# endernewton/tf-faster-rcnn

Hardware: AMD Instinct MI355X
Metric: images/sec (600×1000) ResNet-101 Faster R-CNN at 1/2/4/8 MI355X (higher is better)
Workload: dtype f32 (operands, accumulators, results; GEMMs with Cin, Cout % 128 == 0 form each f32 product from two-piece fp16 operands with an exact power-of-two scale per 128-k block on the fp16 matrix pipe -- 3 MFMAs / product, dropped terms <= 3 * 2^-22, measured error vs float64 below the f32-MFMA kernel's; o

## Files before the change

### include/frcnn_hip.h

```cpp
#ifndef FRCNN_HIP_H_
#define FRCNN_HIP_H_
#include <stddef.h>
#include <stdint.h>

#ifdef __cplusplus
extern "C" {
#endif

#define FRCNN_OK 0
#define FRCNN_E_ARG (-1)
#define FRCNN_E_WS (-2)
#define FRCNN_E_UNSUPPORTED (-3)
#define FRCNN_E_HIP(e) (-(1000 + (int)(e)))

#define FRCNN_NMS_RULE_CPU 0
#define FRCNN_NMS_RULE_GPU 1

#define FRCNN_ACT_NONE 0
#define FRCNN_ACT_RELU 1
#define FRCNN_ACT_RELU6 2

#define FRCNN_ABI_VERSION 6
int frcnn_abi_version(void);
const char* frcnn_build_info(void);
// ... 178 lines not shown
                       const float* res_d, const void* res_planes_d, const float* res_inv_d, int G, int M, int N, int K, int act, int rows,
                       float* mean_out_d, void* ws, size_t ws_bytes, int cfg, void* stream);
int frcnn_winograd_filter_transform(const float* w_hwio, int Cin, int Cout, const float* scale, int m, float* u_out);
int frcnn_winograd_filter_transform_device(const float* w_packed_d, int Cout, int Cin, int m, int transpose_flip, float* u_d,
                                           void* stream);
int frcnn_winograd_input_transform(const float* x_d, int N, int H, int W, int C, int m, float* v_d, void* stream);
int frcnn_winograd_output_transform(const float* m_d, int N, int H, int W, int C, int m, const float* bias_d, int act, float* y_d,
                                    void* stream);
int frcnn_winograd2_conv_x3(const float* x_d, int N, int H, int W, const void* u_planes_d, const float* bias_d, int act, float* y_d,
                            void* stream);
int frcnn_winograd7_filter_transform(const float* w_hwio, int Cin, int Cout, const float* scale, float* u_out);
int frcnn_winograd7_filter_transform_device(const float* w_packed_d, int Cout, int Cin, int transpose_flip, float* u_d, void* stream);
int frcnn_winograd7_input_transform(const float* x_d, int R, int C, float* v_d, void* stream);
int frcnn_winograd7_output_transform(const float* m_d, int R, int C, const float* bias_d, int act, float* y_d, void* stream);
int frcnn_winograd_input_transform_h2(const float* x_d, int N, int H, int W, int C, int m, void* v_planes_d, float* v_inv_d, void* stream);
int frcnn_winograd_output_transform_h2(const float* m_d, int N, int H, int W, int C, int m, const float* bias_d, int act, float* y_d,
                                       void* y_planes_d, float* y_inv_d, void* stream);
int frcnn_winograd7_input_transform_h2(const float* x_d, int R, int C, void* v_planes_d, float* v_inv_d, void* stream);
int frcnn_winograd7_output_transform_h2(const float* m_d, int R, int C, const float* bias_d, int act, float* y_d, void* y_planes_d,
                                        float* y_inv_d, void* stream);
int frcnn_pack_filter_hwio(const float* w_hwio, int KH, int KW, int Cin, int Cout, const float* scale, float* out);
int frcnn_maxpool_nhwc(const float* x_d, int N, int H, int W, int C, int k, int stride, int pad_top,
                       int pad_left, float* y_d, int OH, int OW, void* stream);
int frcnn_dwconv3x3_nhwc(const float* x_d, int N, int H, int W, int C, const float* w_d, const float* bias_d,
                         float* y_d, int OH, int OW, int stride, int pad_top, int pad_left, int act, void* stream);
int frcnn_dwconv3x3_nhwc_h2(const float* x_d, int N, int H, int W, int C, const float* w_d, const float* bias_d, float* y_d,
                            void* y_planes_d, float* y_inv_d, int OH, int OW, int stride, int pad_top, int pad_left, int act, void* stream);
int frcnn_spatial_mean(const float* x_d, int N, int HW, int C, float* y_d, void* stream);
int frcnn_softmax_rows(const float* x_d, int R, int C, int ld, float* y_d, void* stream);
int frcnn_rpn_softmax(const float* score_d, int HW, int A, int ld, float* prob_d, void* stream);
int frcnn_copy_cols(const float* src_d, int R, int ld_src, int col0, int cols, float* dst_d, int ld_dst, void* stream);

size_t frcnn_anchor_target_workspace_bytes(int H, int W, int A, int max_gt);
int frcnn_anchor_target_layer(const float* gt_boxes_d, int G, float im_h, float im_w, int H, int W, int A,
                              int feat_stride, const double* base_d, int rpn_batchsize, double fg_fraction,
                              double pos_overlap, double neg_overlap, long long seed, const double* opts, float* labels_d,
                              float* bbox_targets_d, float* inside_w_d, float* outside_w_d, void* ws,
                              size_t ws_bytes, void* stream);
int frcnn_anchor_target_layer_inject(const float* gt_boxes_d, int G, float im_h, float im_w, int H, int W, int A, int feat_stride,
                                     const double* base_d, int rpn_batchsize, double fg_fraction, double pos_overlap,
                                     double neg_overlap, const int* disable_d, int n_disable, const double* opts, float* labels_d,
                                     float* bbox_targets_d, float* inside_w_d, float* outside_w_d, void* ws, size_t ws_bytes,
                                     void* stream);
int frcnn_proposal_target_layer(const float* rpn_rois_d, const float* rpn_scores_d, int N, const float* gt_boxes_d,
                                int G, int num_classes, int batch_size, double fg_fraction, double fg_thresh,
                                double bg_thresh_hi, double bg_thresh_lo, const double* means4, const double* stds4,
// ... 98 lines not shown
```

### tf-faster-rcnn_amd/csrc/conv_igemm.hip

```cpp
#include "common.h"
#include "mfma_f32.h"
#include <mutex>
#include <type_traits>

__device__ float4 g_zero_page[4];

struct ConvParams {
  const float* x; const float* w; const float* bias; const float* res; float* y;
  const float* mask;
  int N, H, W, Cin, OH, OW, Cout, KH, KW, stride, pad_top, pad_left, act;
  int RH, RW, res_stride;
  int M, Ktot, nsteps;
  int mtiles, ntiles;
  int batch;
  long long gx, gw, gy;
  int reserved;
  int splits, kchunk;
  long long gz;
  int stagger, stagger_slots;
};

__device__ __forceinline__ size_t res_offset_strided(int m, int n, int Cout, int res_stride, int ohow, int OW, int RH, int RW) {
  const int img = m / ohow, rem = m % ohow, oh = rem / OW, ow = rem % OW;
  return ((size_t)(img * RH + oh * res_stride) * RW + ow * res_stride) * Cout + n;
// ... 508 lines not shown
    case IGEMM_64x64_ILV: return launch_conv<64, 64, 32, 32, 2, false, true>(p, st);
    case IGEMM_128_RF: return launch_conv<128, 128, 64, 64, 2, false, false, true>(p, st);
    case IGEMM_128_8W_RF: return launch_conv<128, 128, 32, 64, 2, false, false, true>(p, st);
    case STREAM_64x64: return launch_stream<64, 64, 32, 32, true, false, false>(p, st);
    case STREAM_64x64_RESPF: return launch_stream<64, 64, 32, 32, true, false, true>(p, st);
    case STREAM_128_RF: return launch_stream<128, 128, 64, 64, false, true, false>(p, st);
    case STREAM_128_8W_RF: return launch_stream<128, 128, 32, 64, false, true, false>(p, st);
    case STREAM_128_8W_RF_RESPF: return launch_stream<128, 128, 32, 64, false, true, true>(p, st);
    case STREAM_128x64: return launch_stream<128, 64, 32, 32, true, false, false>(p, st);
    case STREAM_128x64_RESPF: return launch_stream<128, 64, 32, 32, true, false, true>(p, st);
    case STREAM_64x128: return launch_stream<64, 128, 32, 32, true, false, false>(p, st);
    case STREAM_64x128_RESPF: return launch_stream<64, 128, 32, 32, true, false, true>(p, st);
    case STREAM_128x64_4W_RESPF: return launch_stream<128, 64, 64, 32, false, true, true>(p, st);
    case STREAM_64x128_4W_RESPF: return launch_stream<64, 128, 32, 64, false, true, true>(p, st);
    case STREAM_32x64: return launch_stream<32, 64, 32, 32, true, false, false>(p, st);
    case STREAM_32x128: return launch_stream<32, 128, 32, 32, true, false, false>(p, st);
    default: return FRCNN_E_ARG;
  }
}

static thread_local int g_force_cfg = -1, g_stagger = 0, g_stream = 1, g_split_target = 640;
static thread_local int g_plan_images = 0;
static constexpr int PLAN_IMAGES = 4;
extern thread_local int g_wino_rows_below;
extern "C" int frcnn_set_tuning(int key, int value) {
  if (key == 9) { g_wino_rows_below = value > 0 ? value : 256; return FRCNN_OK; }
  if (key == 0) { g_force_cfg = value; return FRCNN_OK; }
  if (key == 5) { g_stagger = value; return FRCNN_OK; }
  if (key == 6) { g_stream = value; return FRCNN_OK; }
  if (key == 7) { g_split_target = value > 0 ? value : 640; return FRCNN_OK; }
  if (key == 8) { g_plan_images = value > 0 ? value : 0; return FRCNN_OK; }
  return FRCNN_E_ARG;
}

static long long plan_rows(long long M) {
  return (g_plan_images > 0 && M % g_plan_images == 0) ? M / g_plan_images * PLAN_IMAGES : M;
}

static long long tiles_128(long long rows, int Cout, int groups) { return (rows + 127) / 128 * cdiv(Cout, 128) * groups; }

static int tile_cfg_64(int Cout) { return Cout > 32 ? IGEMM_64x64_ILV : IGEMM_64x32_NS4; }
static int tile_cfg(long long rows, int Cout, int nsteps, int groups) {
  if (Cout >= 96 && tiles_128(rows, Cout, groups) >= 384 && nsteps >= 8) return Cout >= 1024 ? IGEMM_128_8W_RF : IGEMM_128_RF;
  return tile_cfg_64(Cout);
}

static bool short_k_stream(long long rows, int Cout, int nsteps, int groups) {
  return g_stream && nsteps <= 8 && Cout % 128 == 0 && (rows + 63) / 64 * (Cout / 128) * groups >= 512;
}

static int plan_splits(int M, int Cout, int nsteps) {
  if (g_force_cfg >= 0) return 1;
  M = (int)min(plan_rows(M), (long long)0x7fffffff);
  if (tile_cfg(M, Cout, nsteps, 1) != tile_cfg_64(Cout)) return 1;
// ... 110 lines not shown
                                 int Cout, int KH, int KW, int stride, int pad_top, int pad_left, int act, int fold_w,
                                 void* stream) {
  return conv2d_impl(x_d, N, H, W, Cin, w_d, bias_d, residual_d, RH, RW, res_stride, y_d, OH, OW, Cout, KH, KW, stride, pad_top,
                     pad_left, act, fold_w, nullptr, 0, nullptr, stream);
}

extern "C" int frcnn_conv2d_nhwc_ws(const float* x_d, int N, int H, int W, int Cin, const float* w_d, const float* bias_d,
                                    const float* residual_d, int RH, int RW, int res_stride, float* y_d, int OH, int OW,
                                    int Cout, int KH, int KW, int stride, int pad_top, int pad_left, int act, int fold_w,
                                    void* ws, size_t ws_bytes, void* stream) {
  return conv2d_impl(x_d, N, H, W, Cin, w_d, bias_d, residual_d, RH, RW, res_stride, y_d, OH, OW, Cout, KH, KW, stride, pad_top,
                     pad_left, act, fold_w, ws, ws_bytes, nullptr, stream);
}

extern "C" int frcnn_conv2d_nhwc_masked_ws(const float* x_d, int N, int H, int W, int Cin, const float* w_d, const float* bias_d,
                                           const float* residual_d, int RH, int RW, int res_stride, float* y_d, int OH, int OW,
                                           int Cout, int KH, int KW, int stride, int pad_top, int pad_left, int act, const float* mask_d,
                                           void* ws, size_t ws_bytes, void* stream) {
  if (!mask_d) return FRCNN_E_ARG;
  return conv2d_impl(x_d, N, H, W, Cin, w_d, bias_d, residual_d, RH, RW, res_stride, y_d, OH, OW, Cout, KH, KW, stride, pad_top,
                     pad_left, act, 0, ws, ws_bytes, mask_d, stream);
}

extern "C" int frcnn_gemm_batched_nt(const float* x_d, const float* w_d, float* y_d, int G, int M, int N, int K, void* stream) {
  if (!x_d || !w_d || !y_d || G <= 0 || M <= 0 || N <= 0 || K <= 0) return FRCNN_E_ARG;
  if (K % 32 || G > 65535) return FRCNN_E_UNSUPPORTED;
  ConvParams p = conv_params();
  p.x = x_d; p.w = w_d; p.y = y_d;
  p.N = 1; p.H = 1; p.W = M; p.Cin = K; p.OH = 1; p.OW = M; p.Cout = N;
  p.M = M; p.Ktot = K; p.nsteps = p.kchunk = K / 32;
  p.gx = (long long)M * K; p.gw = (long long)N * K; p.gy = (long long)M * N;
  p.batch = G;
  hipStream_t st = (hipStream_t)stream;
  if (g_force_cfg >= 0) return launch_cfg(g_force_cfg, p, st);
  const long long Mp = plan_rows(M);
  if (short_k_stream(Mp, N, p.nsteps, G)) {
    const int rc = launch_cfg(STREAM_64x128, p, st);
    if (rc != FRCNN_E_UNSUPPORTED) return rc;
  }
  const bool waste = (Mp + 127) / 128 * 128 * 4 > Mp * 5;
  return launch_cfg(waste ? tile_cfg_64(N) : tile_cfg(Mp, N, p.nsteps, G), p, st);
}

extern "C" int frcnn_pack_filter_hwio(const float* w_hwio, int KH, int KW, int Cin, int Cout, const float* scale, float* out) {
  if (!w_hwio || !out || KH <= 0 || KW <= 0 || Cin <= 0 || Cout <= 0) return FRCNN_E_ARG;
  for (int kh = 0; kh < KH; ++kh)
// ... 9 lines not shown
```

### tf-faster-rcnn_amd/frcnn_hip/__init__.py

```python
import ctypes
import os
from ctypes import c_double, c_float, c_int, c_longlong, c_size_t, c_ulonglong, c_void_p

_PKG = os.path.dirname(os.path.abspath(__file__))
LIB_PATH = os.path.join(_PKG, "libfrcnn_hip.so")
_lib = None

ABI_VERSION = 6
ACT_NONE, ACT_RELU, ACT_RELU6 = 0, 1, 2
NMS_RULE_CPU, NMS_RULE_GPU = 0, 1

_P = c_void_p
SIGNATURES = {
    "frcnn_abi_version": (c_int, []),
    "frcnn_build_info": (ctypes.c_char_p, []),
    "_nms": (None, [_P, _P, _P, c_int, c_int, c_float, c_int]),
    "frcnn_nms_workspace_bytes": (c_size_t, [c_int]),
    "frcnn_nms": (c_int, [_P, c_int, c_double, c_int, _P, _P, _P, c_size_t, _P]),
    "frcnn_nms_sorted": (c_int, [_P, c_int, c_int, c_double, c_int, _P, _P, _P, c_size_t, _P]),
    "frcnn_nms_rule": (c_int, [_P, c_int, c_double, c_int, c_int, _P, _P, _P, c_size_t, _P]),
    "frcnn_nms_sorted_rule": (c_int, [_P, c_int, c_int, c_double, c_int, c_int, _P, _P, _P, c_size_t, _P]),
    "frcnn_generate_anchors": (c_int, [c_int, _P, c_int, _P, c_int, _P]),
    "frcnn_generate_anchors_pre": (c_int, [c_int, c_int, c_int, _P, c_int, _P, _P]),
    "frcnn_proposal_workspace_bytes": (c_size_t, [c_int, c_int, c_int, c_int]),
# ... 69 lines not shown
    "frcnn_jpeg_coefs": (c_int, [_P, c_int, c_int, c_int, c_int, c_int, _P, _P, c_size_t, _P]),
    "frcnn_jpeg_coefs_host": (c_int, [_P, c_int, c_int, c_int, c_int, c_int, _P]),
    "frcnn_jpeg_stream_bound": (c_size_t, [c_int, c_int, c_int, c_int]),
    "frcnn_jpeg_entropy_encode": (c_longlong, [_P, c_int, c_int, c_int, c_int, _P, c_size_t]),
    "frcnn_draw_detections": (c_int, [_P, c_int, c_int, _P, _P, c_int, c_float, c_int, c_int, _P, c_int, _P, c_int, c_int, _P, _P]),
    "frcnn_draw_detections_host": (c_int, [_P, c_int, c_int, _P, c_int, c_int, c_float, c_int, c_int, _P, c_int, _P, c_int, c_int, _P]),
    "frcnn_gemm_batched_nt": (c_int,[_P, _P, _P, c_int, c_int, c_int, c_int, _P]),
    "frcnn_winograd_filter_transform": (c_int, [_P, c_int, c_int, _P, c_int, _P]),
    "frcnn_winograd_filter_transform_device": (c_int, [_P, c_int, c_int, c_int, c_int, _P, _P]),
    "frcnn_winograd_input_transform": (c_int, [_P, c_int, c_int, c_int, c_int, c_int, _P, _P]),
    "frcnn_winograd_output_transform": (c_int, [_P, c_int, c_int, c_int, c_int, c_int, _P, c_int, _P, _P]),
    "frcnn_winograd2_conv_x3": (c_int, [_P, c_int, c_int, c_int, _P, _P, c_int, _P, _P]),
    "frcnn_winograd7_filter_transform": (c_int, [_P, c_int, c_int, _P, _P]),
    "frcnn_winograd7_filter_transform_device": (c_int, [_P, c_int, c_int, c_int, _P, _P]),
    "frcnn_winograd7_input_transform": (c_int, [_P, c_int, c_int, _P, _P]),
    "frcnn_winograd7_output_transform": (c_int, [_P, c_int, c_int, _P, c_int, _P, _P]),
    "frcnn_winograd_input_transform_h2": (c_int, [_P, c_int, c_int, c_int, c_int, c_int, _P, _P, _P]),
    "frcnn_winograd_output_transform_h2": (c_int, [_P, c_int, c_int, c_int, c_int, c_int, _P, c_int, _P, _P, _P, _P]),
    "frcnn_winograd7_input_transform_h2": (c_int, [_P, c_int, c_int, _P, _P, _P]),
    "frcnn_winograd7_output_transform_h2": (c_int, [_P, c_int, c_int, _P, c_int, _P, _P, _P, _P]),
    "frcnn_set_tuning": (c_int, [c_int, c_int]),
    "frcnn_pack_filter_hwio": (c_int, [_P, c_int, c_int, c_int, c_int, _P, _P]),
    "frcnn_maxpool_nhwc": (c_int, [_P, c_int, c_int, c_int, c_int, c_int, c_int, c_int, c_int, _P, c_int, c_int, _P]),
    "frcnn_dwconv3x3_nhwc": (c_int, [_P, c_int, c_int, c_int, c_int, _P, _P, _P, c_int, c_int, c_int, c_int, c_int, c_int, _P]),
    "frcnn_dwconv3x3_nhwc_h2": (c_int, [_P, c_int, c_int, c_int, c_int, _P, _P, _P, _P, _P, c_int, c_int, c_int, c_int, c_int, c_int, _P]),
    "frcnn_spatial_mean": (c_int, [_P, c_int, c_int, c_int, _P, _P]),
    "frcnn_softmax_rows": (c_int, [_P, c_int, c_int, c_int, _P, _P]),
    "frcnn_rpn_softmax": (c_int, [_P, c_int, c_int, c_int, _P, _P]),
    "frcnn_copy_cols": (c_int, [_P, c_int, c_int, c_int, c_int, _P, c_int, _P]),
    "frcnn_anchor_target_workspace_bytes": (c_size_t, [c_int, c_int, c_int, c_int]),
    "frcnn_anchor_target_layer": (c_int, [_P, c_int, c_float, c_float, c_int, c_int, c_int, c_int, _P, c_int, c_double, c_double,
                                          c_double, c_longlong, _P, _P, _P, _P, _P, _P, c_size_t, _P]),
    "frcnn_anchor_target_layer_inject": (c_int, [_P, c_int, c_float, c_float, c_int, c_int, c_int, c_int, _P, c_int, c_double, c_double,
                                                 c_double, _P, c_int, _P, _P, _P, _P, _P, _P, c_size_t, _P]),
    "frcnn_proposal_target_layer_inject": (c_int, [_P, _P, c_int, _P, c_int, c_int, c_int, _P, c_int, _P, _P, _P, _P, _P, _P, _P, _P, _P, _P]),
    "frcnn_proposal_target_layer": (c_int, [_P, _P, c_int, _P, c_int, c_int, c_int, c_double, c_double, c_double, c_double, _P, _P,
                                            c_longlong, _P, _P, _P, _P, _P, _P, _P, _P, _P]),
    "frcnn_proposal_target_layer_dn": (c_int, [_P, _P, c_int, _P, _P, c_int, c_int, c_int, c_double, c_double, c_double, c_double, _P, _P,
                                               c_longlong, _P, _P, _P, _P, _P, _P, _P, _P, _P]),
    "frcnn_loss_workspace_bytes": (c_size_t, [c_longlong]),
    "frcnn_softmax_ce_loss": (c_int, [_P, _P, c_int, c_int, c_int, c_int, c_int, _P, _P, _P, c_size_t, _P]),
    "frcnn_smooth_l1_loss": (c_int, [_P, _P, _P, _P, c_longlong, c_float, c_float, _P, _P, _P, c_size_t, _P]),
    "frcnn_transpose_pad": (c_int, [_P, c_int, c_int, _P, c_int, _P]),
    "frcnn_im2col_t": (c_int, [_P, c_int, c_int, c_int, c_int, c_int, c_int, c_int, c_int, c_int, c_int, c_int, _P, c_int, _P]),
    "frcnn_flip_transpose_filter": (c_int, [_P, c_int, c_int, c_int, c_int, _P, _P]),
    "frcnn_conv2d_dgrad_strided": (c_int, [_P, c_int, c_int, c_int, c_int, _P, c_int, c_int, c_int, c_int, c_int, c_int, _P, c_int,
# ... 87 lines not shown
```

### tf-faster-rcnn_amd/frcnn_hip/ops.py

```python
import ctypes

import numpy as np
import torch

import frcnn_hip as _binding
from . import ACT_NONE, NMS_RULE_CPU, call, check, lib

_ws_cache = {}
ws_scope = "default"

_scope_stack = [(None, None, None)]


def active_store(owner, default=None):
    o, _, store = _scope_stack[-1]
    return store if store is not None and (owner is None or o is owner) else default


def scope_depth():
    return len(_scope_stack) - 1


class unscoped(object):

# ... 875 lines not shown
        v = _empty((G, T, Cin), dtype=torch.float32, device=dev) if v_buf is None else v_buf
        winograd_input_transform(x, v, m)
        gemm_batched_nt(v, u, mm)
    if mask is not None:
        assert bias is None and act == ACT_NONE
        return winograd_output_transform_masked(mm, mask, out, m, out_planes)
    if out_planes is not None:
        winograd_output_transform_h2(mm, bias, act, tuple(out.shape), m, out_planes, out)
        return out
    return winograd_output_transform(mm, bias, act, out, m)


def maxpool(x, k, stride, pad=(0, 0, 0, 0), out=None):
    _chk(x)
    N, H, W, C = x.shape
    OH = conv_out_size(H, k, stride, pad[0], pad[1])
    OW = conv_out_size(W, k, stride, pad[2], pad[3])
    out = _empty((N, OH, OW, C), dtype=torch.float32, device=x.device) if out is None else out
    call("frcnn_maxpool_nhwc", _ptr(x), N, H, W, C, int(k), int(stride), int(pad[0]), int(pad[2]), _ptr(out), OH, OW,
         _stream())
    return out


def dwconv3x3(x, w, bias, stride=1, pad=(1, 1, 1, 1), act=ACT_NONE, out=None, out_planes=None, want_f32=True):
    _chk(x), _chk(w)
    N, H, W, C = x.shape
    OH = conv_out_size(H, 3, stride, pad[0], pad[1])
    OW = conv_out_size(W, 3, stride, pad[2], pad[3])
    if out_planes is None:
        out = _empty((N, OH, OW, C), dtype=torch.float32, device=x.device) if out is None else out
        call("frcnn_dwconv3x3_nhwc", _ptr(x), N, H, W, C, _ptr(w), _ptr(bias), _ptr(out), OH, OW, int(stride),
             int(pad[0]), int(pad[2]), int(act), _stream())
        return out
    assert isinstance(out_planes, H2) and out_planes.rows == N * OH * OW and out_planes.K == C
    if want_f32 and out is None:
        out = _empty((N, OH, OW, C), dtype=torch.float32, device=x.device)
    call("frcnn_dwconv3x3_nhwc_h2", _ptr(x), N, H, W, C, _ptr(w), _ptr(bias), _ptr(out if want_f32 else None), _ptr(out_planes.planes),
         _ptr(out_planes.inv), OH, OW, int(stride), int(pad[0]), int(pad[2]), int(act), _stream())
    return out if want_f32 else None


def spatial_mean(x, out=None):
    _chk(x)
    N, C = x.shape[0], x.shape[-1]
    HW = x.numel() // (N * C)
    out = _empty((N, C), dtype=torch.float32, device=x.device) if out is None else out
# ... 505 lines not shown
```

### tf-faster-rcnn_amd/frcnn_hip/replay.py

```python
import ctypes
import time

import torch


class Arena(object):

    def __init__(self, sess, tag):
        self.sess, self.tag, self.n = sess, tag, 0

    def reset(self):
        self.n = 0

    def take(self, shape, dtype, device):
        key = ("arena", self.tag, self.n, tuple(int(s) for s in shape), dtype)
        self.n += 1
        store = self.sess._store()
        t = store.get(key)
        if t is None:
            t = store[key] = torch.empty(key[3], dtype=dtype, device=self.sess.device if device is None else device)
        return t


class Recording(object):
# ... 137 lines not shown
        s = (time.perf_counter() - self.t0) / self.window
        self.log.append(("inherited" if self.cur is None else "slot %d -> pool[%d]" % self.cur, s))
        if self.best_s is None or s < self.best_s * (1.0 - self.gain):
            self.best_s = s
            if self.cur is not None:
                self.best[self.cur[0]] = self.pool[self.cur[1]]
        if not self.queue:
            self._finish(main)

    def _finish(self, main):
        b = list(self.best)
        b[0] = main
        self.rec.bind(b)
        self.done = True


NO_STREAM_ARG = frozenset(["frcnn_set_tuning", "frcnn_detect_set_tuning", "frcnn_conv2d_wgrad_set_plan", "frcnn_conv2d_wgrad_h2_set_plan"])
HOST_ONLY = frozenset(["frcnn_generate_anchors", "frcnn_winograd_filter_transform", "frcnn_winograd7_filter_transform", "frcnn_pack_filter_hwio",
                       "frcnn_prep_image_shape", "frcnn_crc32c", "frcnn_snappy_uncompress", "_nms", "frcnn_graph_begin", "frcnn_graph_end",
                       "frcnn_graph_launch", "frcnn_graph_destroy", "frcnn_abi_version", "frcnn_build_info", "frcnn_sgd_desc_bytes",
                       "frcnn_conv2d_wgrad_supported", "frcnn_jpeg_info", "frcnn_jpeg_entropy_decode", "frcnn_jpeg_pixels_host", "frcnn_summary_limits",
                       "frcnn_jpeg_quant_tables", "frcnn_jpeg_coefs_host", "frcnn_jpeg_stream_bound", "frcnn_jpeg_entropy_encode",
                       "frcnn_draw_detections_host", "frcnn_proposal_recall_host", "frcnn_soft_nms_host",
                       "frcnn_box_vote_host", "frcnn_merge_flip_views_host"])
```

### tf-faster-rcnn_amd/lib/model/config.py

```python
import ast
import os
import os.path as osp

import numpy as np


class AttrDict(dict):

    def __init__(self, d=None, **kw):
        super().__init__()
        for k, v in dict(d or {}, **kw).items():
            self[k] = v

    def __setitem__(self, k, v):
        if isinstance(v, dict) and not isinstance(v, AttrDict):
            v = AttrDict(v)
        super().__setitem__(k, v)

    def __getattr__(self, k):
        try:
            return self[k]
        except KeyError:
            raise AttributeError(k)

# ... 7 lines not shown
    FG_FRACTION=0.25, FG_THRESH=0.5, BG_THRESH_HI=0.5, BG_THRESH_LO=0.1, USE_FLIPPED=True, BBOX_REG=True,
    BBOX_THRESH=0.5, SNAPSHOT_ITERS=5000, SNAPSHOT_PREFIX='res101_faster_rcnn', BBOX_NORMALIZE_TARGETS=True,
    BBOX_INSIDE_WEIGHTS=(1.0, 1.0, 1.0, 1.0), BBOX_NORMALIZE_TARGETS_PRECOMPUTED=True,
    BBOX_NORMALIZE_MEANS=(0.0, 0.0, 0.0, 0.0), BBOX_NORMALIZE_STDS=(0.1, 0.1, 0.2, 0.2), PROPOSAL_METHOD='gt',
    HAS_RPN=True, RPN_POSITIVE_OVERLAP=0.7, RPN_NEGATIVE_OVERLAP=0.3, RPN_CLOBBER_POSITIVES=False,
    RPN_FG_FRACTION=0.5, RPN_BATCHSIZE=256, RPN_NMS_THRESH=0.7, RPN_PRE_NMS_TOP_N=12000,
    RPN_POST_NMS_TOP_N=2000, RPN_BBOX_INSIDE_WEIGHTS=(1.0, 1.0, 1.0, 1.0), RPN_POSITIVE_WEIGHT=-1.0,
    USE_ALL_GT=True)

_TEST = dict(
    SCALES=(600,), MAX_SIZE=1000, NMS=0.3, SVM=False, BBOX_REG=True, HAS_RPN=False, PROPOSAL_METHOD='gt',
    RPN_NMS_THRESH=0.7, RPN_PRE_NMS_TOP_N=6000, RPN_POST_NMS_TOP_N=300, MODE='nms', RPN_TOP_N=5000)

__C = AttrDict(
    TRAIN=_TRAIN, TEST=_TEST,
    RESNET=dict(MAX_POOL=False, FIXED_BLOCKS=1),
    MOBILENET=dict(REGU_DEPTH=False, FIXED_LAYERS=5, WEIGHT_DECAY=0.00004, DEPTH_MULTIPLIER=1.),
    PIXEL_MEANS=np.array([[[102.9801, 115.9465, 122.7717]]]), RNG_SEED=3,
    ROOT_DIR=osp.abspath(osp.join(osp.dirname(__file__), '..', '..')),
    MATLAB='matlab', EXP_DIR='default', USE_GPU_NMS=True, USE_E2E_TF=False, POOLING_MODE='crop', POOLING_SIZE=7,
    ANCHOR_SCALES=[8, 16, 32], ANCHOR_RATIOS=[0.5, 1, 2], RPN_CHANNELS=512,
    HIP=dict(WINOGRAD=True, WINOGRAD_MIN_CIN=64, WINOGRAD_M=4, WINOGRAD_F2_SCOPES=("block1", "block2"), WINOGRAD_DIRECT_SCOPES=(),
             WINOGRAD_TRAIN=True, WINOGRAD_DGRAD=True,
             WINOGRAD_7X7=True, WINOGRAD_FUSED_F2=True, FUSE_TAIL_MEAN=True, MFMA_X3=True,
             MFMA_H2=True, H2_LAZY_SPLIT=True, H2_MIN_TILES=150, H2_TRAIN_MIN_TILES=320, H2_TRUNK_PLANES=True, H2_TILE_CFG=-1,
             X3_TILE_CFG=-1, H2_TRAIN=True, WGRAD_STREAM=2, WGRAD_TN=True, WGRAD_H2=True, PREP_STREAM=True, TRAIN_REPLAY=True, TRAIN_PICK_STREAMS=6,
             GRAPH_CACHE_SHAPES=4, TRAIN_CACHE_SHAPES=16, JPEG_DEVICE=False, TEST_BATCH_IMAGES=1,
             SOFT_NMS=0, SOFT_NMS_SIGMA=0.5, SOFT_NMS_MIN_SCORE=0.001, TEST_FLIP=False, BBOX_VOTE=False, BBOX_VOTE_THRESH=0.8))
__C.DATA_DIR = osp.abspath(osp.join(__C.ROOT_DIR, 'data'))
cfg = __C


def get_output_dir(imdb, weights_filename):
    outdir = osp.abspath(osp.join(__C.ROOT_DIR, 'output', __C.EXP_DIR, imdb.name))
    outdir = osp.join(outdir, 'default' if weights_filename is None else weights_filename)
    os.makedirs(outdir, exist_ok=True)
    return outdir


def get_output_tb_dir(imdb, weights_filename):
    outdir = osp.abspath(osp.join(__C.ROOT_DIR, 'tensorboard', __C.EXP_DIR, imdb.name))
    outdir = osp.join(outdir, 'default' if weights_filename is None else weights_filename)
    os.makedirs(outdir, exist_ok=True)
    return outdir


_NULLABLE_KEYS = ("H2_TRAIN_MIN_TILES",)
# ... 59 lines not shown
```

### tf-faster-rcnn_amd/lib/nets/network.py

```python
import collections

import numpy as np
import torch

from frcnn_hip import ACT_NONE, ACT_RELU, NMS_RULE_CPU, NMS_RULE_GPU, ops
from frcnn_hip.runtime import VarSpec
from model.config import cfg


class Network(object):
    def __init__(self):
        self._predictions = {}
        self._losses = {}
        self._anchor_targets = {}
        self._proposal_targets = {}
        self._layers = {}
        self._act_summaries = []
        self._variables_to_fix = {}
        self._feat_stride = [16, ]
        self._scope = "network"
        self._sess = None
        self._image = None
        self._im_info = None
        self._var_specs = collections.OrderedDict()
# ... 560 lines not shown
        self._var(self._scope + "/bbox_pred/biases", (4 * num_classes,), "zeros")
        names = ["rois", "rpn_cls_score", "rpn_cls_prob", "rpn_bbox_pred", "cls_score", "cls_prob", "bbox_pred"]
        return {k: k for k in names}

    def _stage_image(self, sess, image, im_info=None):
        if isinstance(image, np.ndarray):
            image = torch.from_numpy(np.ascontiguousarray(image, dtype=np.float32))
        B, H, W, C = image.shape
        if im_info is None:
            buf = sess.buf(self._tag + "/image", (B, H, W, 4), zero=True)
        else:
            with self.shape_scope(sess, (B, H, W, 4), im_info):
                buf = sess.buf(self._tag + "/image", (B, H, W, 4), zero=True)
        buf[..., :C].copy_(image, non_blocking=True)
        return buf

    def graph_key(self, image_shape, im_info):
        c = cfg[self._mode]
        return (self._tag, self._scope, self._num_classes, self._anchor_scales, self._anchor_ratios, bool(cfg.RESNET.MAX_POOL),
                bool(cfg.USE_GPU_NMS), tuple(int(v) for v in image_shape), (float(im_info[0]), float(im_info[1])), self._mode, cfg.TEST.MODE, self._fuse_tail_entry,
                c.RPN_PRE_NMS_TOP_N, c.RPN_POST_NMS_TOP_N, c.RPN_NMS_THRESH, cfg.TEST.RPN_TOP_N, cfg.POOLING_SIZE,
                bool(cfg.HIP.WINOGRAD), int(cfg.HIP.WINOGRAD_MIN_CIN), int(cfg.HIP.WINOGRAD_M), tuple(cfg.HIP.WINOGRAD_F2_SCOPES),
                tuple(cfg.HIP.WINOGRAD_DIRECT_SCOPES), bool(cfg.HIP.WINOGRAD_7X7), bool(cfg.HIP.FUSE_TAIL_MEAN), bool(cfg.HIP.MFMA_X3), bool(cfg.USE_E2E_TF),
                bool(cfg.HIP.MFMA_H2), bool(cfg.HIP.H2_LAZY_SPLIT), int(cfg.HIP.H2_MIN_TILES), bool(cfg.HIP.H2_TRUNK_PLANES), int(cfg.HIP.H2_TILE_CFG), int(cfg.HIP.X3_TILE_CFG), bool(cfg.HIP.H2_TRAIN))

    def shape_scope(self, sess, image_shape, im_info):
        return sess.shape_scope(self.graph_key(image_shape, im_info), group=("graphs", self._tag), cap=int(cfg.HIP.GRAPH_CACHE_SHAPES))

    def forward_device(self, sess, image_d, im_info, use_graph=True):
        self._sess = sess
        self._image = image_d
        self._im_info = (float(im_info[0]), float(im_info[1]), float(im_info[2]))
        sess.prepared.wait_planes()
        ops.ws_scope = self._tag
        key = self.graph_key(image_d.shape, self._im_info)
        cur = torch.cuda.current_stream(sess.device)
        with self.shape_scope(sess, image_d.shape, self._im_info):
            if not use_graph or sess.profile is not None:
                sess.flops_last_forward = 0
                self._build_network(self._mode == "TRAIN")
                return self._predictions
            if key not in sess.graphs:
                with torch.cuda.stream(sess.stream):
                    sess.stream.wait_stream(cur)
                    sess.flops_last_forward = 0
                    self._build_network(False)
                    sess.stream.synchronize()
# ... 406 lines not shown
```

### tf-faster-rcnn_amd/lib/nets/resnet_v1.py

```python
from frcnn_hip import ACT_NONE, ACT_RELU, ops
from model.config import cfg
from nets.network import Network

BN_EPS = 1e-5


def _same_pad(k, stride):
    total = k - 1
    beg = total // 2
    return (beg, total - beg, beg, total - beg)


class resnetv1(Network):
    _rgb_first_conv = "/conv1"
    _trainable_on_device = True
    def __init__(self, num_layers=50):
        Network.__init__(self)
        self._feat_stride = [16, ]
        self._feat_compress = [1. / float(self._feat_stride[0]), ]
        self._num_layers = num_layers
        self._scope = 'resnet_v1_%d' % num_layers
        self._decide_blocks()

    def _decide_blocks(self):
# ... 51 lines not shown

    def _trunk_planes_only(self, rows, base, next_stride, next_prefix=None):
        depth = 4 * base
        return (bool(cfg.HIP.H2_TRUNK_PLANES) and next_stride == 1
                and self._h2_eligible(rows, base, depth, 1, None if next_prefix is None else next_prefix + "/conv1")
                and self._h2_eligible(rows, depth, base, 1, None if next_prefix is None else next_prefix + "/conv3"))

    def _run_blocks(self, x, blocks, emit_last=True):
        for bi, (name, base, n_units, stride) in enumerate(blocks):
            for u in range(1, n_units + 1):
                s_u = stride if u == n_units else 1
                N, H, W, _ = x.shape
                rows = N * ops.conv_out_size(H, 3, s_u, 1, 1) * ops.conv_out_size(W, 3, s_u, 1, 1) if s_u > 1 else N * H * W
                planes_only = u < n_units and self._trunk_planes_only(rows, base, stride if u + 1 == n_units else 1,
                                                                       "%s/%s/unit_%d/bottleneck_v1" % (self._scope, name, u + 1))
                x = self._bottleneck(x, "%s/%s/unit_%d/bottleneck_v1" % (self._scope, name, u), base, s_u,
                                     emit_out=emit_last or u < n_units or bi + 1 < len(blocks), f32_out=not planes_only)
        return x

    def _crop_pool_layer(self, bottom, rois, name):
        return self._crop_pool(bottom, rois, name, max_pool=bool(cfg.RESNET.MAX_POOL))

    def _build_base(self):
        net = self._conv(self._image, self._scope + "/conv1", 7, 2, _same_pad(7, 2), act=ACT_RELU, bn_eps=BN_EPS,
                         fold_w=True, real_cin=3)
        N, H, W, C = net.shape
        out = self._sess.buf(self._tag + "/pool1", (N, ops.conv_out_size(H, 3, 2, 1, 1), ops.conv_out_size(W, 3, 2, 1, 1), C))
        self._sess.mark("op:maxpool", 0, lambda: ops.maxpool(net, 3, 2, (1, 1, 1, 1), out=out), nbytes=4 * (net.numel() + out.numel()))
        return self._wrote(out)

    def _image_to_head(self, is_training, reuse=None):
        assert (0 <= cfg.RESNET.FIXED_BLOCKS <= 3)
        net_conv = self._run_blocks(self._build_base(), self._blocks[0:3])
        self._act_summaries.append(net_conv)
        self._layers['head'] = net_conv
        return net_conv

    def _fused_tail_maps(self, net_conv):
        name = self._blocks[-1][0]
        prefix = "%s/%s/unit_1/bottleneck_v1" % (self._scope, name)
        sc_map = self._conv(net_conv, prefix + "/shortcut", 1, 1, act=ACT_NONE, bn_eps=BN_EPS, no_bias=True)
        c1_map = self._conv(net_conv, prefix + "/conv1", 1, 1, act=ACT_NONE, bn_eps=BN_EPS, no_bias=True)
        return sc_map, c1_map

    def _fused_tail_entry(self, net_conv, rois):
        sess, P = self._sess, cfg.POOLING_SIZE
# ... 50 lines not shown
```

Before: 554.5.

## Fuse stem 7x7 conv with 3x3 max-pool in one MFMA kernel for inference

Adds a dedicated kernel that computes the conv1 7x7/stride-2 convolution on f32 MFMAs, then applies bias, ReLU and the 3x3/stride-2 max-pool from LDS, writing only the pooled output. This removes the full-resolution conv1 activation write and its re-read by the separate maxpool. By default it also skips the MFMA for the padded fourth input channel (DROP3). A heuristic picks the segment height so the tail wave of blocks is balanced. The trade-off is more LDS, more barriers per step, and halo rows recomputed at segment borders.

```diff
diff --git a/include/frcnn_hip.h b/include/frcnn_hip.h
--- a/include/frcnn_hip.h
+++ b/include/frcnn_hip.h
@@ -224,6 +224,9 @@
 int frcnn_pack_filter_hwio(const float* w_hwio, int KH, int KW, int Cin, int Cout, const float* scale, float* out);
 int frcnn_maxpool_nhwc(const float* x_d, int N, int H, int W, int C, int k, int stride, int pad_top,
                        int pad_left, float* y_d, int OH, int OW, void* stream);
+int frcnn_stem_conv_pool(const float* x_d, int N, int H, int W, const float* w_foldw_d, const float* bias_d, float* y_d, int PH, int PW,
+                         void* stream);
+int frcnn_stem_conv_pool_tiling(int N, int PH, int PW, int* strip_pw, int* seg_ph);
 int frcnn_dwconv3x3_nhwc(const float* x_d, int N, int H, int W, int C, const float* w_d, const float* bias_d,
                          float* y_d, int OH, int OW, int stride, int pad_top, int pad_left, int act, void* stream);
 int frcnn_dwconv3x3_nhwc_h2(const float* x_d, int N, int H, int W, int C, const float* w_d, const float* bias_d, float* y_d,
diff --git a/scratch/stem_pool_time.py b/scratch/stem_pool_time.py
--- /dev/null
+++ b/scratch/stem_pool_time.py
@@ -0,0 +1,67 @@
+import os
+import sys
+
+import numpy as np
+import torch
+
+ROOT = os.path.dirname(os.path.dirname(os.path.abspath(__file__)))
+for p in (ROOT, os.path.join(ROOT, "tf-faster-rcnn_amd"), os.path.join(ROOT, "tf-faster-rcnn_amd", "lib")):
+    sys.path.insert(0, p)
+from frcnn_hip import ACT_RELU, call, ops
+
+args = [a for a in sys.argv[1:] if not a.startswith("--")]
+N, H, W = (int(v) for v in args[:3]) if len(args) >= 3 else (8, 600, 1000)
+segs = [int(v) for v in sys.argv[sys.argv.index("--segs") + 1].split(",")] if "--segs" in sys.argv else []
+dev = torch.device("cuda:0")
+rng = np.random.RandomState(1)
+x = np.zeros((N, H, W, 4), np.float32)
+x[..., :3] = rng.randn(N, H, W, 3).astype(np.float32) * 50
+x = torch.from_numpy(x).to(dev)
+w = torch.from_numpy(ops.pack_filter_foldw((rng.randn(7, 7, 3, 64) * 0.05).astype(np.float32))).to(dev)
+b = torch.from_numpy(rng.randn(64).astype(np.float32)).to(dev)
+PH, PW = ops.stem_pool_shape(H, W)
+conv = torch.empty((N, (H - 1) // 2 + 1, (W - 1) // 2 + 1, 64), device=dev)
+pool = torch.empty((N, PH, PW, 64), device=dev)
+fused = torch.empty_like(pool)
+
+
+def fused_route(keep_e3, seg_ph):
+    def f():
+        call("frcnn_set_tuning", 10, keep_e3)
+        call("frcnn_set_tuning", 11, seg_ph)
+        ops.stem_conv_pool(x, w, b, out=fused)
+        call("frcnn_set_tuning", 10, 0)
+        call("frcnn_set_tuning", 11, 0)
+    return f
+
+
+routes = [("conv1", lambda: ops.conv2d(x, w, b, 7, 7, 2, (3, 3, 3, 3), ACT_RELU, fold_w=True, out=conv)),
+          ("pool1", lambda: ops.maxpool(conv, 3, 2, (1, 1, 1, 1), out=pool)),
+          ("fused", fused_route(0, 0)), ("fused + e==3 MFMAs", fused_route(1, 0))]
+routes += [("fused, segments of %d" % s, fused_route(0, s)) for s in segs]
+print("shape", (N, H, W), "strip width, segment height:", ops.stem_conv_pool_tiling(N, PH, PW))
+for _, f in routes:
+    f()
+torch.cuda.synchronize()
+print("fused == conv1 + pool1, bit for bit:", torch.equal(fused.view(torch.int32), pool.view(torch.int32)))
+ROUNDS, WARM = 50, 3
+times = {n: [] for n, _ in routes}
+for r in range(ROUNDS + WARM):
+    evs = []
+    for n, f in routes:
+        e0, e1 = torch.cuda.Event(enable_timing=True), torch.cuda.Event(enable_timing=True)
+        e0.record()
+        f()
+        e1.record()
+        evs.append((n, e0, e1))
+    torch.cuda.synchronize()
+    if r >= WARM:
+        for n, e0, e1 in evs:
+            times[n].append(e0.elapsed_time(e1) * 1000.0)
+print("%-26s %9s %9s %9s %9s" % ("launch (us)", "median", "min", "p10", "p90"))
+for n, _ in routes:
+    t = np.array(times[n])
+    print("%-26s %9.1f %9.1f %9.1f %9.1f" % (n, np.median(t), t.min(), np.percentile(t, 10), np.percentile(t, 90)))
+s = np.array(times["conv1"]) + np.array(times["pool1"])
+print("%-26s %9.1f %9.1f %9.1f %9.1f   sum of medians %.1f" % ("conv1 + pool1 (per round)", np.median(s), s.min(), np.percentile(s, 10), np.percentile(s, 90),
+                                                               np.median(times["conv1"]) + np.median(times["pool1"])))
diff --git a/tf-faster-rcnn_amd/csrc/conv_igemm.hip b/tf-faster-rcnn_amd/csrc/conv_igemm.hip
--- a/tf-faster-rcnn_amd/csrc/conv_igemm.hip
+++ b/tf-faster-rcnn_amd/csrc/conv_igemm.hip
@@ -554,6 +554,7 @@
 static thread_local int g_force_cfg = -1, g_stagger = 0, g_stream = 1, g_split_target = 640;
 static thread_local int g_plan_images = 0;
 static constexpr int PLAN_IMAGES = 4;
+static thread_local int g_stem_keep_e3 = 0, g_stem_seg_ph = 0;
 extern thread_local int g_wino_rows_below;
 extern "C" int frcnn_set_tuning(int key, int value) {
   if (key == 9) { g_wino_rows_below = value > 0 ? value : 256; return FRCNN_OK; }
@@ -562,6 +563,8 @@
   if (key == 6) { g_stream = value; return FRCNN_OK; }
   if (key == 7) { g_split_target = value > 0 ? value : 640; return FRCNN_OK; }
   if (key == 8) { g_plan_images = value > 0 ? value : 0; return FRCNN_OK; }
+  if (key == 10) { g_stem_keep_e3 = value != 0; return FRCNN_OK; }
+  if (key == 11) { g_stem_seg_ph = value > 0 ? value : 0; return FRCNN_OK; }
   return FRCNN_E_ARG;
 }
 
@@ -718,6 +721,209 @@
                      pad_left, act, 0, ws, ws_bytes, mask_d, stream);
 }
 
+struct StemParams {
+  const float* x; const float* w; const float* bias; float* y;
+  int N, H, W, OH, OW, PH, PW;
+  int strips, segs, seg_ph;
+};
+static constexpr int STEM_STRIP_PW = 15, STEM_SEG_PH = 25, STEM_SEG_PH_MIN = 5, STEM_FILL = 512;
+
+typedef float f32x4 __attribute__((ext_vector_type(4)));
+__device__ __forceinline__ void gstore16(float* dst, float4 v) {
+  const f32x4 d = {v.x, v.y, v.z, v.w};
+  asm volatile("global_store_dwordx4 %0, %1, off" ::"v"(dst), "v"(d) : "memory");
+}
+__device__ __forceinline__ float4 fmax4(float4 a, float4 b) { return make_float4(fmaxf(a.x, b.x), fmaxf(a.y, b.y), fmaxf(a.z, b.z), fmaxf(a.w, b.w)); }
+
+template <bool DROP3>
+__global__ __launch_bounds__(256) void k_stem_conv_pool(const StemParams p) {
+  constexpr int BM = 128, NS = 3, P = NS - 1, LA = 4, LB = 2, G = LA + LB, KH = 7;
+  constexpr int SLAB = (BM + 64) * 32;
+  extern __shared__ __attribute__((aligned(16))) float smem[];
+  float* const tile = smem + SLAB;
+
+  const int tid = threadIdx.x, lane = tid & 63;
+  const int wave = __builtin_amdgcn_readfirstlane(tid >> 6);
+  int bid = blockIdx.x;
+  const int strip = bid % p.strips; bid /= p.strips;
+  const int img = bid % p.N, seg = bid / p.N;
+  const int k0 = seg * p.seg_ph, kend = min(k0 + p.seg_ph, p.PH);
+  const int nsteps = (kend - k0) / 2 + 1;
+  const int ow0 = strip * (2 * STEM_STRIP_PW) - 1;
+
+  const int lrow = lane >> 3, lpos = lane & 7;
+  const float* zero = (const float*)g_zero_page;
+  int a_off[LA]; bool a_ok[LA];
+#pragma unroll
+  for (int t = 0; t < LA; ++t) {
+    const int row = (wave * LA + t) * 8 + lrow;
+    const int iw = (ow0 + (row & 31)) * 2 - 3 + (lpos ^ ((row >> 1) & 7));
+    a_ok[t] = (unsigned)iw < (unsigned)p.W;
+    a_off[t] = (img * p.H * p.W + iw) * 4;
+  }
+  const float* b_ptr[LB];
+#pragma unroll
+  for (int t = 0; t < LB; ++t) {
+    const int row = BM + (wave * LB + t) * 8 + lrow;
+    b_ptr[t] = p.w + (row - BM) * (KH * 32) + (lpos ^ ((row >> 1) & 7)) * 4;
+  }
+  const unsigned lds0 = (unsigned)(size_t)(LDS_AS float*)smem;
+  auto issue_slab = [&](int kh, int buf, int ih0) {
+    const int ih = ih0 + kh;
+    const bool rok = (unsigned)ih < (unsigned)p.H;
+    const unsigned sb = lds0 + (unsigned)(buf * SLAB * 4);
+#pragma unroll
+    for (int t = 0; t < LA; ++t)
+      glds16(rok && a_ok[t] ? p.x + (a_off[t] + ih * p.W * 4) : zero, __builtin_amdgcn_readfirstlane(sb + (wave * LA + t) * 1024));
+#pragma unroll
+    for (int t = 0; t < LB; ++t) glds16(b_ptr[t] + kh * 32, __builtin_amdgcn_readfirstlane(sb + BM * 128 + (wave * LB + t) * 1024));
+  };
+
+  const int frow = lane & 31, khalf = lane >> 5;
+  int koff[4];
+#pragma unroll
+  for (int s = 0; s < 4; ++s) koff[s] = ((2 * s + khalf) ^ ((frow >> 1) & 7)) * 4;
+  const int a_row0 = (wave * 32 + frow) * 32, b_row0 = (BM + frow) * 32;
+
+  const int pc = tid >> 4, c4 = (tid & 15) * 4;
+  const int pw = strip * STEM_STRIP_PW + pc;
+  const bool pool_lane = pc < STEM_STRIP_PW && pw < p.PW;
+  float4 bv = *(const float4*)(p.bias + c4);
+  asm volatile("" : "+v"(bv.x), "+v"(bv.y), "+v"(bv.z), "+v"(bv.w));
+  const float4 ninf = make_float4(-INFINITY, -INFINITY, -INFINITY, -INFINITY);
+  float4 c0 = ninf, c1 = ninf;
+  auto emit = [&](int ph, float4 m) {
+    if (ph < k0 || ph >= kend) return;
+    if (2 * ph - 1 < 0 || 2 * ph + 1 >= p.OH || 2 * pw - 1 < 0 || 2 * pw + 1 >= p.OW) m = fmax4(m, make_float4(0.f, 0.f, 0.f, 0.f));
+    gstore16(p.y + (((size_t)img * p.PH + ph) * p.PW + pw) * 64 + c4, m);
+  };
+
+  int r0 = 2 * k0 - 1;
+  issue_slab(0, 0, (r0 + wave) * 2 - 3);
+  issue_slab(1, 1, (r0 + wave) * 2 - 3);
+  for (int i = 0; i < nsteps; ++i, r0 += 4) {
+    const int ih0 = (r0 + wave) * 2 - 3;
+    f32x16 acc[2];
+#pragma unroll
+    for (int j = 0; j < 2; ++j)
+#pragma unroll
+      for (int r = 0; r < 16; ++r) acc[j][r] = 0.f;
+#pragma unroll
+    for (int kh = 0; kh < KH; ++kh) {
+      if (kh + P <= KH) wait_vmcnt<(P - 1) * G>();
+      else wait_vmcnt<0>();
+      __builtin_amdgcn_s_barrier();
+      const float* sb = smem + (kh % NS) * SLAB;
+      if (kh + P < KH) issue_slab(kh + P, (kh + P) % NS, ih0);
+      float4 a[4][1], b[4][2];
+#pragma unroll
+      for (int q = 0; q < 4; ++q) frag_read(a[q], sb, a_row0, koff[q], b[q], b_row0);
+#pragma unroll
+      for (int q = 0; q < 4; ++q)
+#pragma unroll
+        for (int e = 0; e < (DROP3 ? 3 : 4); ++e)
+#pragma unroll
+          for (int j = 0; j < 2; ++j) {
+            const float av = e == 0 ? a[q][0].x : e == 1 ? a[q][0].y : e == 2 ? a[q][0].z : a[q][0].w;
+            const float bw = e == 0 ? b[q][j].x : e == 1 ? b[q][j].y : e == 2 ? b[q][j].z : b[q][j].w;
+            acc[j] = __builtin_amdgcn_mfma_f32_32x32x2f32(av, bw, acc[j], 0, 0, 0);
+          }
+    }
+    __syncthreads();
+    const bool more = i + 1 < nsteps;
+    if (more) issue_slab(0, 0, ih0 + 8);
+#pragma unroll
+    for (int j = 0; j < 2; ++j)
+#pragma unroll
+      for (int r = 0; r < 16; ++r) tile[(wave * 32 + (r & 3) + 8 * (r >> 2) + 4 * khalf) * 64 + j * 32 + frow] = acc[j][r];
+    __syncthreads();
+    float4 v[4][3];
+#pragma unroll
+    for (int tr = 0; tr < 4; ++tr)
+#pragma unroll
+      for (int d = 0; d < 3; ++d) v[tr][d] = *(const float4*)(tile + (tr * 32 + min(2 * pc + d, 31)) * 64 + c4);
+#pragma unroll
+    for (int tr = 0; tr < 4; ++tr)
+      asm volatile("" : "+v"(v[tr][0].x), "+v"(v[tr][0].y), "+v"(v[tr][0].z), "+v"(v[tr][0].w), "+v"(v[tr][1].x), "+v"(v[tr][1].y),
+                   "+v"(v[tr][1].z), "+v"(v[tr][1].w), "+v"(v[tr][2].x), "+v"(v[tr][2].y), "+v"(v[tr][2].z), "+v"(v[tr][2].w));
+    float4 h[4];
+#pragma unroll
+    for (int tr = 0; tr < 4; ++tr) {
+      float4 m = ninf;
+      const bool rok = pool_lane && (unsigned)(r0 + tr) < (unsigned)p.OH;
+#pragma unroll
+      for (int d = 0; d < 3; ++d) {
+        float4 t = v[tr][d];
+        t.x += bv.x; t.y += bv.y; t.z += bv.z; t.w += bv.w;
+        t = act_relu(t);
+        const float4 mt = fmax4(m, t);
+        if (rok && (unsigned)(ow0 + 2 * pc + d) < (unsigned)p.OW) m = mt;
+      }
+      h[tr] = m;
+    }
+    __syncthreads();
+    if (more) issue_slab(1, 1, ih0 + 8);
+    if (pool_lane) {
+      emit(k0 + 2 * i - 1, fmax4(fmax4(c0, c1), h[0]));
+      emit(k0 + 2 * i, fmax4(fmax4(h[0], h[1]), h[2]));
+    }
+    c0 = h[2]; c1 = h[3];
+  }
+}
+
+static int stem_seg_ph(int N, int PH, int PW) {
+  if (g_stem_seg_ph > 0) return g_stem_seg_ph;
+  const long long cols = (long long)N * cdiv(PW, STEM_STRIP_PW);
+  long long best = 0;
+  int best_s = STEM_SEG_PH;
+  for (int S = STEM_SEG_PH; S >= STEM_SEG_PH_MIN; S -= 2) {
+    const int segs = cdiv(PH, S);
+    const long long a = 2 * (S / 2 + 1) + 1, b = 2 * ((PH - (segs - 1) * S) / 2 + 1) + 1;
+    const long long nfull = cols * (segs - 1), r = nfull / STEM_FILL, rem = nfull % STEM_FILL;
+    const long long span_full = (rem ? r + 1 : r) * a;
+    const long long on_idle = r * a + (cols + STEM_FILL - rem - 1) / (STEM_FILL - rem) * b;
+    const long long on_top = span_full + (cols + STEM_FILL - 1) / STEM_FILL * b;
+    const long long span = max(span_full, min(on_idle, on_top));
+    if (S == STEM_SEG_PH || span < best) { best = span; best_s = S; }
+  }
+  return best_s;
+}
+
+extern "C" int frcnn_stem_conv_pool_tiling(int N, int PH, int PW, int* strip_pw, int* seg_ph) {
+  if (N <= 0 || PH <= 0 || PW <= 0 || !strip_pw || !seg_ph) return FRCNN_E_ARG;
+  *strip_pw = STEM_STRIP_PW;
+  *seg_ph = stem_seg_ph(N, PH, PW);
+  return FRCNN_OK;
+}
+
+extern "C" int frcnn_stem_conv_pool(const float* x_d, int N, int H, int W, const float* w_foldw_d, const float* bias_d, float* y_d, int PH,
+                                    int PW, void* stream) {
+  if (!x_d || !w_foldw_d || !bias_d || !y_d) return FRCNN_E_ARG;
+  if (N <= 0 || H <= 0 || W <= 0 || PH <= 0 || PW <= 0) return FRCNN_E_ARG;
+  const int OH = (H - 1) / 2 + 1, OW = (W - 1) / 2 + 1;
+  if (PH != (OH - 1) / 2 + 1 || PW != (OW - 1) / 2 + 1) return FRCNN_E_ARG;
+  if ((long long)N * H * W * 4 >= (1ll << 31) || (long long)N * OH * OW >= (1ll << 31) / 4) return FRCNN_E_UNSUPPORTED;
+  StemParams p;
+  p.x = x_d; p.w = w_foldw_d; p.bias = bias_d; p.y = y_d;
+  p.N = N; p.H = H; p.W = W; p.OH = OH; p.OW = OW; p.PH = PH; p.PW = PW;
+  p.seg_ph = stem_seg_ph(N, PH, PW);
+  p.strips = cdiv(PW, STEM_STRIP_PW);
+  p.segs = cdiv(PH, p.seg_ph);
+  constexpr size_t lds = sizeof(float) * 3 * (128 + 64) * 32;
+  const dim3 grid((unsigned)(N * p.strips * p.segs));
+  if (g_stem_keep_e3) {
+    static KernelOnce once;
+    HIP_TRY(kernel_once(once, (const void*)k_stem_conv_pool<false>, 256, lds));
+    hipLaunchKernelGGL(k_stem_conv_pool<false>, grid, dim3(256), lds, (hipStream_t)stream, p);
+  } else {
+    static KernelOnce once;
+    HIP_TRY(kernel_once(once, (const void*)k_stem_conv_pool<true>, 256, lds));
+    hipLaunchKernelGGL(k_stem_conv_pool<true>, grid, dim3(256), lds, (hipStream_t)stream, p);
+  }
+  LAUNCH_CHECK();
+  return FRCNN_OK;
+}
+
 extern "C" int frcnn_gemm_batched_nt(const float* x_d, const float* w_d, float* y_d, int G, int M, int N, int K, void* stream) {
   if (!x_d || !w_d || !y_d || G <= 0 || M <= 0 || N <= 0 || K <= 0) return FRCNN_E_ARG;
   if (K % 32 || G > 65535) return FRCNN_E_UNSUPPORTED;
diff --git a/tf-faster-rcnn_amd/frcnn_hip/__init__.py b/tf-faster-rcnn_amd/frcnn_hip/__init__.py
--- a/tf-faster-rcnn_amd/frcnn_hip/__init__.py
+++ b/tf-faster-rcnn_amd/frcnn_hip/__init__.py
@@ -115,6 +115,8 @@
     "frcnn_set_tuning": (c_int, [c_int, c_int]),
     "frcnn_pack_filter_hwio": (c_int, [_P, c_int, c_int, c_int, c_int, _P, _P]),
     "frcnn_maxpool_nhwc": (c_int, [_P, c_int, c_int, c_int, c_int, c_int, c_int, c_int, c_int, _P, c_int, c_int, _P]),
+    "frcnn_stem_conv_pool": (c_int, [_P, c_int, c_int, c_int, _P, _P, _P, c_int, c_int, _P]),
+    "frcnn_stem_conv_pool_tiling": (c_int, [c_int, c_int, c_int, _P, _P]),
     "frcnn_dwconv3x3_nhwc": (c_int, [_P, c_int, c_int, c_int, c_int, _P, _P, _P, c_int, c_int, c_int, c_int, c_int, c_int, _P]),
     "frcnn_dwconv3x3_nhwc_h2": (c_int, [_P, c_int, c_int, c_int, c_int, _P, _P, _P, _P, _P, c_int, c_int, c_int, c_int, c_int, c_int, _P]),
     "frcnn_spatial_mean": (c_int, [_P, c_int, c_int, c_int, _P, _P]),
diff --git a/tf-faster-rcnn_amd/frcnn_hip/ops.py b/tf-faster-rcnn_amd/frcnn_hip/ops.py
--- a/tf-faster-rcnn_amd/frcnn_hip/ops.py
+++ b/tf-faster-rcnn_amd/frcnn_hip/ops.py
@@ -921,6 +921,30 @@
     return out
 
 
+def stem_pool_shape(H, W):
+    return (conv_out_size(conv_out_size(H, 7, 2, 3, 3), 3, 2, 1, 1), conv_out_size(conv_out_size(W, 7, 2, 3, 3), 3, 2, 1, 1))
+
+
+def stem_conv_pool_tiling(N, PH, PW):
+    sw, sh = ctypes.c_int(), ctypes.c_int()
+    call("frcnn_stem_conv_pool_tiling", int(N), int(PH), int(PW), ctypes.byref(sw), ctypes.byref(sh))
+    return sw.value, sh.value
+
+
+def stem_conv_pool(x, w_foldw, bias, out=None):
+    if x.dim() != 4 or x.shape[3] != 4 or tuple(w_foldw.shape) != (64, 7, 8, 4) or tuple(bias.shape) != (64,):
+        raise ValueError("stem_conv_pool: x [N,H,W,4], w_foldw [64,7,8,4], bias [64]; got %s %s %s"
+                         % (tuple(x.shape), tuple(w_foldw.shape), tuple(bias.shape)))
+    _chk(x), _chk(w_foldw), _chk(bias)
+    N, H, W, C = x.shape
+    PH, PW = stem_pool_shape(H, W)
+    out = _empty((N, PH, PW, 64), dtype=torch.float32, device=x.device) if out is None else out
+    if tuple(out.shape) != (N, PH, PW, 64):
+        raise ValueError("stem_conv_pool: out must be %s, got %s" % ((N, PH, PW, 64), tuple(out.shape)))
+    call("frcnn_stem_conv_pool", _ptr(x), N, H, W, _ptr(w_foldw), _ptr(bias), _ptr(out), PH, PW, _stream())
+    return out
+
+
 def dwconv3x3(x, w, bias, stride=1, pad=(1, 1, 1, 1), act=ACT_NONE, out=None, out_planes=None, want_f32=True):
     _chk(x), _chk(w)
     N, H, W, C = x.shape
diff --git a/tf-faster-rcnn_amd/frcnn_hip/replay.py b/tf-faster-rcnn_amd/frcnn_hip/replay.py
--- a/tf-faster-rcnn_amd/frcnn_hip/replay.py
+++ b/tf-faster-rcnn_amd/frcnn_hip/replay.py
@@ -183,4 +183,4 @@
                        "frcnn_conv2d_wgrad_supported", "frcnn_jpeg_info", "frcnn_jpeg_entropy_decode", "frcnn_jpeg_pixels_host", "frcnn_summary_limits",
                        "frcnn_jpeg_quant_tables", "frcnn_jpeg_coefs_host", "frcnn_jpeg_stream_bound", "frcnn_jpeg_entropy_encode",
                        "frcnn_draw_detections_host", "frcnn_proposal_recall_host", "frcnn_soft_nms_host",
-                       "frcnn_box_vote_host", "frcnn_merge_flip_views_host"])
+                       "frcnn_box_vote_host", "frcnn_merge_flip_views_host", "frcnn_stem_conv_pool_tiling"])
diff --git a/tf-faster-rcnn_amd/lib/model/config.py b/tf-faster-rcnn_amd/lib/model/config.py
--- a/tf-faster-rcnn_amd/lib/model/config.py
+++ b/tf-faster-rcnn_amd/lib/model/config.py
@@ -53,7 +53,7 @@
     ANCHOR_SCALES=[8, 16, 32], ANCHOR_RATIOS=[0.5, 1, 2], RPN_CHANNELS=512,
     HIP=dict(WINOGRAD=True, WINOGRAD_MIN_CIN=64, WINOGRAD_M=4, WINOGRAD_F2_SCOPES=("block1", "block2"), WINOGRAD_DIRECT_SCOPES=(),
              WINOGRAD_TRAIN=True, WINOGRAD_DGRAD=True,
-             WINOGRAD_7X7=True, WINOGRAD_FUSED_F2=True, FUSE_TAIL_MEAN=True, MFMA_X3=True,
+             WINOGRAD_7X7=True, WINOGRAD_FUSED_F2=True, STEM_FUSED_POOL=True, FUSE_TAIL_MEAN=True, MFMA_X3=True,
              MFMA_H2=True, H2_LAZY_SPLIT=True, H2_MIN_TILES=150, H2_TRAIN_MIN_TILES=320, H2_TRUNK_PLANES=True, H2_TILE_CFG=-1,
              X3_TILE_CFG=-1, H2_TRAIN=True, WGRAD_STREAM=2, WGRAD_TN=True, WGRAD_H2=True, PREP_STREAM=True, TRAIN_REPLAY=True, TRAIN_PICK_STREAMS=6,
              GRAPH_CACHE_SHAPES=4, TRAIN_CACHE_SHAPES=16, JPEG_DEVICE=False, TEST_BATCH_IMAGES=1,
diff --git a/tf-faster-rcnn_amd/lib/nets/network.py b/tf-faster-rcnn_amd/lib/nets/network.py
--- a/tf-faster-rcnn_amd/lib/nets/network.py
+++ b/tf-faster-rcnn_amd/lib/nets/network.py
@@ -606,7 +606,8 @@
                 c.RPN_PRE_NMS_TOP_N, c.RPN_POST_NMS_TOP_N, c.RPN_NMS_THRESH, cfg.TEST.RPN_TOP_N, cfg.POOLING_SIZE,
                 bool(cfg.HIP.WINOGRAD), int(cfg.HIP.WINOGRAD_MIN_CIN), int(cfg.HIP.WINOGRAD_M), tuple(cfg.HIP.WINOGRAD_F2_SCOPES),
                 tuple(cfg.HIP.WINOGRAD_DIRECT_SCOPES), bool(cfg.HIP.WINOGRAD_7X7), bool(cfg.HIP.FUSE_TAIL_MEAN), bool(cfg.HIP.MFMA_X3), bool(cfg.USE_E2E_TF),
-                bool(cfg.HIP.MFMA_H2), bool(cfg.HIP.H2_LAZY_SPLIT), int(cfg.HIP.H2_MIN_TILES), bool(cfg.HIP.H2_TRUNK_PLANES), int(cfg.HIP.H2_TILE_CFG), int(cfg.HIP.X3_TILE_CFG), bool(cfg.HIP.H2_TRAIN))
+                bool(cfg.HIP.MFMA_H2), bool(cfg.HIP.H2_LAZY_SPLIT), int(cfg.HIP.H2_MIN_TILES), bool(cfg.HIP.H2_TRUNK_PLANES), int(cfg.HIP.H2_TILE_CFG), int(cfg.HIP.X3_TILE_CFG), bool(cfg.HIP.H2_TRAIN),
+                bool(cfg.HIP.STEM_FUSED_POOL))
 
     def shape_scope(self, sess, image_shape, im_info):
         return sess.shape_scope(self.graph_key(image_shape, im_info), group=("graphs", self._tag), cap=int(cfg.HIP.GRAPH_CACHE_SHAPES))
diff --git a/tf-faster-rcnn_amd/lib/nets/resnet_v1.py b/tf-faster-rcnn_amd/lib/nets/resnet_v1.py
--- a/tf-faster-rcnn_amd/lib/nets/resnet_v1.py
+++ b/tf-faster-rcnn_amd/lib/nets/resnet_v1.py
@@ -97,6 +97,17 @@
         return self._crop_pool(bottom, rois, name, max_pool=bool(cfg.RESNET.MAX_POOL))
 
     def _build_base(self):
+        if cfg.HIP.STEM_FUSED_POOL and self._mode == "TEST":
+            scope = self._scope + "/conv1"
+            x, sess = self._image, self._sess
+            w, b = sess.conv_params(scope, bn_eps=BN_EPS, fold_w=True)
+            self._need_f32(x)
+            N, H, W, _ = x.shape
+            PH, PW = ops.stem_pool_shape(H, W)
+            out = sess.buf(self._tag + "/pool1", (N, PH, PW, w.shape[0]))
+            flops = 2 * N * ops.conv_out_size(H, 7, 2, 3, 3) * ops.conv_out_size(W, 7, 2, 3, 3) * w.shape[0] * 7 * 7 * 3
+            sess.mark("conv:" + scope, flops, lambda: ops.stem_conv_pool(x, w, b, out=out), nbytes=4 * (x.numel() + w.numel() + out.numel()))
+            return self._wrote(out)
         net = self._conv(self._image, self._scope + "/conv1", 7, 2, _same_pad(7, 2), act=ACT_RELU, bn_eps=BN_EPS,
                          fold_w=True, real_cin=3)
         N, H, W, C = net.shape
```

Result: no change. 558.4, median of 6 (+0.7%).
